# TeemoCaption/FDDM-asr

Measured on AMD Instinct MI355X. Metric: train-step utterances/sec (10 s @16 kHz, seq_len 256) at 1/2/4/8 MI355X, higher is better.
Workload: dtype bf16; 1 GPU; fddm_zhTW_base C2: WavLM-base + 6L d512 H8 ff2048 decoder, V=8000, T=200, dropout 0.1, n_step_fd=4; global_batch=32, seq_len=256, parallelism=dp1

## Files before the change

fddm-asr_amd/fddm_hip/graphs.py:

```python
from __future__ import annotations

import weakref
from types import SimpleNamespace

import torch

from . import runtime as rt


class GraphedEncoder:
    def __init__(self, encoder, nslots: int = 2):
        self._enc = weakref.ref(encoder)
        self.nslots = nslots
        self.cache: dict = {}

    @staticmethod
    def supported(encoder) -> bool:
        return getattr(encoder, "pooling", "none") == "none" and hasattr(encoder, "backbone") and \
            hasattr(encoder.backbone, "stage_rest")

    @property
    def enc(self):
        return self._enc()

    def _capture(self, wave):
        bb = self.enc.backbone
        inp = wave.detach().clone()
        h0 = bb.stage_conv0(inp)
        h1 = bb.stage_conv1(h0)
        self.enc.project(bb.stage_rest(h1))
        with rt.retaining() as keep:
            gA = torch.cuda.CUDAGraph()
            with torch.cuda.graph(gA):
                h0 = bb.stage_conv0(inp)
            h1 = torch.empty(bb.conv_out_shape(h0), device=h0.device, dtype=h0.dtype)
            gC = torch.cuda.CUDAGraph()
            with torch.cuda.graph(gC, pool=gA.pool()):
                out = self.enc.project(bb.stage_rest(h1))
        return SimpleNamespace(inp=inp, h0=h0, h1=h1, out=out, gA=gA, gC=gC, keep=keep)

    def _weights_token(self):
        enc = self.enc
        P = enc.backbone._prepared(rt.compute_dtype())
        proj = getattr(enc, "proj", None)
        pw = getattr(proj, "weight", None) if getattr(enc, "use_proj", False) else None
        return (id(P), None if pw is None else (pw.data_ptr(), pw._version), rt.cache_epoch()), P

    @torch.no_grad()
    def run(self, wave, slot: int, cap: int = 0):
        tok, P = self._weights_token()
        if tok != getattr(self, "_tok", None):
            self.cache.clear()
            self._tok, self._P = tok, P
        key = (tuple(wave.shape), wave.dtype, str(wave.device), rt.precision(), int(cap),
               int(getattr(self.enc.backbone, "conv_cus", 0)),
               int(getattr(self.enc.backbone, "conv_cus_rest", 0)))
        slots = self.cache.setdefault(key, [None] * self.nslots)
        s = slots[slot]
        if s is None:
            s = slots[slot] = self._capture(wave)
        s.inp.copy_(wave, non_blocking=True)
        s.gA.replay()
        self.enc.backbone.stage_conv1(s.h0, out=s.h1)
        s.gC.replay()
        return s.out


class StepGraphs:

    def __init__(self, device):
        self.device = torch.device(device)
        self.graphs: dict = {}
        self.static: dict = {}
        self.pool = None
        self.off = torch.zeros(1, device=self.device, dtype=torch.int64)

    def reset(self):
        self.graphs.clear()
        self.static.clear()
        self.pool = None

    @staticmethod
    def _hparams(optimizer):
        return tuple((float(g.get("lr", 0.0)), float(g.get("weight_decay", 0.0)),
                      tuple(float(b) for b in g.get("betas", ())), float(g.get("eps", 0.0)))
                     for g in getattr(optimizer, "param_groups", ()))

    def _token(self, params, optimizer, step_args):
        return (rt.cache_epoch(), getattr(optimizer, "table_epoch", 0), self._hparams(optimizer), tuple(step_args),
                tuple((p.data_ptr(), p._version) for p in params))

    def get(self, kind, params, optimizer, shapes, step_args=()):
        s = self.graphs.get(kind)
        if s is None:
            return None
        if s.shapes != shapes or s.token != self._token(params, optimizer, step_args):
            self.reset()
            return None
        return s

    def capture(self, kind, fn, inputs: dict, params, optimizer, step_args=()):
        from ._lib import lib
        shapes = tuple((k, tuple(v.shape), v.dtype) for k, v in sorted(inputs.items()))
        if any(self.static.get(k) is None or self.static[k].shape != v.shape or self.static[k].dtype != v.dtype
               for k, v in inputs.items()):
            self.reset()
            self.static = {k: torch.empty_like(v) for k, v in inputs.items()}
        for k, v in inputs.items():
            self.static[k].copy_(v)
        c0 = rt.seed_counter()
        g = torch.cuda.CUDAGraph()
        with rt.retaining() as keep:
            lib().fddm_set_seed_offset(self.off.data_ptr())
            try:
                with torch.cuda.graph(g, pool=self.pool):
                    outs = fn(**self.static)
            finally:
                lib().fddm_set_seed_offset(None)
        nseeds = rt.seed_counter() - c0
        rt.set_seed_counter(c0)
        if self.pool is None:
            self.pool = g.pool()
        self.graphs[kind] = SimpleNamespace(g=g, outs=outs, c0=c0, nseeds=nseeds, keep=keep, shapes=shapes,
                                            token=self._token(params, optimizer, step_args))

    def replay(self, kind, inputs: dict):
        s = self.graphs[kind]
        for k, v in inputs.items():
            self.static[k].copy_(v, non_blocking=True)
        c = rt.seed_counter()
        self.off.fill_(c - s.c0)
        rt.set_seed_counter(c + s.nseeds)
        s.g.replay()
        return s.outs
```

fddm-asr_amd/fddm_hip/runtime.py:

```python
from __future__ import annotations

import contextlib
import math
import os

import weakref

import torch

from . import ops

_precision = os.environ.get("FDDM_PRECISION", "bf16")


def precision() -> str:
    return _precision


def set_precision(p: str) -> None:
    global _precision
    if p not in ("bf16", "fp32"):
        raise ValueError(p)
    _precision = p

# ... 145 lines not shown


def set_seed_counter(c: int) -> None:
    global _seed_counter
    _seed_counter = int(c)


def reseed(seed: int) -> None:
    global _base_seed, _seed_counter
    _base_seed = int(seed) & 0xFFFFFFFF
    _seed_counter = 0


def seed_state() -> list:
    return [-1 if _base_seed is None else int(_base_seed), int(_seed_counter)]


def set_seed_state(state) -> None:
    global _base_seed, _seed_counter
    b, c = int(state[0]), int(state[1])
    _base_seed = None if b < 0 else b
    _seed_counter = c


_tables: dict = {}


def _table_get(k, owner):
    v = _tables.get(k)
    return _retain(v[1]) if v is not None and v[0]() is owner else None


def _table_put(k, owner, t):
    _tables[k] = (weakref.ref(owner), _retain(t))


def rope_tables(L: int, inv_freq: torch.Tensor, device):
    k = ("rope", L, id(inv_freq), inv_freq._version, inv_freq.numel(), str(device))
    t = _table_get(k, inv_freq)
    if t is None:
        f = inv_freq.detach().float().cpu()
        pos = torch.arange(L, dtype=f.dtype)
        fr = torch.outer(pos, f)
        emb = torch.cat((fr, fr), dim=-1)
        t = (emb.cos().contiguous().to(device), emb.sin().contiguous().to(device))
        _table_put(k, inv_freq, t)
    return t


def rel_bucket(rel: torch.Tensor, num_buckets: int, max_distance: int) -> torch.Tensor:
    nb = num_buckets // 2
    buckets = (rel > 0).to(torch.long) * nb
    rel = torch.abs(rel)
    max_exact = nb // 2
    is_small = rel < max_exact
    large = torch.log(rel.float() / max_exact)
    large = large / math.log(max_distance / max_exact)
    large = large * (nb - max_exact)
    large = (max_exact + large).to(torch.long)
    large = torch.min(large, torch.full_like(large, nb - 1))
    return buckets + torch.where(is_small, rel, large)


def relbias_table(S: int, embed: torch.Tensor, num_buckets: int, max_distance: int):
    k = ("rel", S, id(embed), embed._version, num_buckets, max_distance)
    t = _table_get(k, embed)
    if t is None:
        rel = torch.arange(-(S - 1), S)
        b = rel_bucket(rel, num_buckets, max_distance).to(embed.device)
        t = embed.detach().float()[b].t().contiguous()
        _table_put(k, embed, t)
    return t


class GradArena:

    ALIGN = 64

    def __init__(self, params, order=None):
        self.params = [p for p in params if p.requires_grad]
        if not self.params:
            raise ValueError("empty grad arena")
        if order is not None:
            rank = {id(p): i for i, p in enumerate(order)}
            self.params.sort(key=lambda p: rank.get(id(p), len(rank)))
        offs, n = [], 0
        for p in self.params:
            offs.append(n)
            n += (p.numel() + self.ALIGN - 1) // self.ALIGN * self.ALIGN
        dev = self.params[0].device
        self.flat = torch.zeros(n, device=dev, dtype=torch.float32)
        self.offs = offs + [n]
        self.slot = {id(p): i for i, p in enumerate(self.params)}
        self.on_ready = None
        self.reducer = None
        self.clean = False
        self.views = []
        for p, o in zip(self.params, offs):
            v = self.flat[o:o + p.numel()].view_as(p)
            self.views.append(v)
            p._fddm_arena = self
        self.attach()

    def attach(self):
        for p, v in zip(self.params, self.views):
            if p.grad is None or p.grad.data_ptr() != v.data_ptr():
                p.grad = v

    def zero_(self):
        self.attach()
        self.flat.zero_()


def grads_ready(params) -> None:
    for p in params:
        a = getattr(p, "_fddm_arena", None)
        if a is not None and a.on_ready is not None:
            a.on_ready(params)
            return


def grad_slot(p: torch.Tensor):
    a = getattr(p, "_fddm_arena", None)
    g = p.grad
    if a is None or g is None or g.dtype != torch.float32:
        return None
    return g


_probes: dict | None = None
_replay_n = 0


@contextlib.contextmanager
def probe(name: str, replay=None):
    if _probes is None or name not in _probes:
        yield
        return
    s = torch.cuda.current_stream()
    e0, e1 = torch.cuda.Event(enable_timing=True), torch.cuda.Event(enable_timing=True)
    e0.record(s)
    yield
    e1.record(s)
    _probes[name].append((e0, e1))
    if replay is not None and _replay_n > 0:
        r0, r1 = torch.cuda.Event(enable_timing=True), torch.cuda.Event(enable_timing=True)
        r0.record(s)
        for _ in range(_replay_n):
            replay()
        r1.record(s)
        _probes.setdefault(name + "#replay", []).append((r0, r1, _replay_n))


def probing_any(prefix: str) -> bool:
    return _probes is not None and any(n.startswith(prefix) for n in _probes)


@contextlib.contextmanager
def probing(names, replays=0):
    global _probes, _replay_n
    old, old_n = _probes, _replay_n
    _probes = {n: [] for n in names}
    _replay_n = replays
    try:
        yield _probes
    finally:
        _probes, _replay_n = old, old_n
```

fddm-asr_amd/train.py:

```python
from __future__ import annotations

import argparse
import logging
import os
import random
import time
import weakref
from dataclasses import dataclass
from datetime import datetime

import torch
import yaml

from fddm.sched.diffusion_scheduler import DiscreteDiffusionScheduler
from fddm_hip import dist as fdist
from fddm_hip import functions as FN
from fddm_hip import runtime as rt
from fddm_hip._lib import lib as _fddm_lib
from fddm_hip.graphs import GraphedEncoder, StepGraphs
from fddm_hip.optim import FusedAdamW
from losses.fddm_losses import lfd_loss
from models.acoustic_encoder import AcousticEncoder
from models.denoise_decoder import DenoisingTransformerDecoder
from models.projection import SpeechProjector, TextEmbedding, TextProjector

try:
    from tqdm import tqdm
except Exception:
    tqdm = None


@dataclass
class Config:
    seed: int
    data: dict
    model: dict
    diffusion: dict
    inference: dict
    optim: dict
    lfd: dict
    log: dict


class SchedulerAdapter:

    def __init__(self, scheduler):
        self.sch = scheduler

    def sample_q(self, x0: torch.Tensor, t: torch.Tensor) -> torch.Tensor:
        if hasattr(self.sch, "sample_xt"):
            return self.sch.sample_xt(x0, t, rt.next_seed())
        B, L = x0.shape
        onehot = torch.zeros(B, L, self.sch.K, device=x0.device)
        onehot.scatter_(-1, x0.unsqueeze(-1), 1.0)
        p = self.sch.q_sample(onehot, t)
        return torch.multinomial(p.view(-1, self.sch.K), 1).view(B, L)

    def kl_term(self, xt, x0, logits_x0, t, x_mask=None) -> torch.Tensor:
        if not hasattr(self.sch, "betas"):
            raise ValueError("scheduler must provide betas [T] to build the posterior")
        mask = None
        if x_mask is not None:
            mask = x_mask.contiguous().view(torch.uint8) if x_mask.dtype == torch.bool else \
                (x_mask != 0).contiguous().view(torch.uint8)
            mask = mask.reshape(-1)
        betas = self.sch.betas
        if betas.device != logits_x0.device or betas.dtype != torch.float32:
            betas = betas.to(logits_x0.device).float().contiguous()
        return FN.KLFn.apply(logits_x0.float(), xt, x0, t, mask, betas)

    def w_t(self, t: torch.Tensor) -> torch.Tensor:
        if hasattr(self.sch, "alpha_bar"):
            return self.sch.alpha_bar.to(t.device)[t - 1]
        if hasattr(self.sch, "w_prefix"):
            return self.sch.w_prefix.to(t.device)[t - 1]
        if hasattr(self.sch, "betas"):
            cp = torch.cumprod(1.0 - self.sch.betas.to(t.device), 0)
            return cp[t - 1]
        return torch.ones_like(t, dtype=torch.float32)


def align_speech(z_speech: torch.Tensor, L: int) -> torch.Tensor:
    S = z_speech.size(1)
    if S >= L:
        return z_speech[:, :L, :]
    return torch.cat([z_speech, z_speech[:, -1:, :].repeat(1, L - S, 1)], dim=1)


def cu_caps(dev) -> dict:
    ncu = torch.cuda.get_device_properties(dev).multi_processor_count
    coll = int(os.environ.get("FDDM_COLL_CUS", 0))
    enc = int(os.environ.get("FDDM_ENC_CUS", ncu * 3 // 4))
    conv = int(os.environ.get("FDDM_ENC_CUS_CONV", ncu // 2))
    conv_rest = int(os.environ.get("FDDM_ENC_CUS_CONV2", conv))
    low = lambda c: max(8, c - coll)
    return {"enc": low(enc), "conv": low(conv), "conv_rest": low(conv_rest), "coll": coll, "ncu": ncu}


def _encoded(encoder, loader, device, optimizer):
    opt_ids = set(id(p) for g in optimizer.param_groups for p in g["params"])
    frozen = not any(id(p) in opt_ids for p in encoder.parameters())
    dev = torch.device(device)
    if dev.type != "cuda" or not frozen or os.environ.get("FDDM_NO_ENC_PIPELINE"):
        bb = getattr(encoder, "backbone", None)
        if bb is not None and getattr(bb, "conv_cus", 0):
            bb.conv_cus = bb.conv_cus_rest = 0
        for wave, x0, *rest in loader:
            wave = wave.to(device, non_blocking=True)
            x0 = x0.to(device, non_blocking=True)
            if rest and rest[0] is not None:
                c, c_mask, _ = encoder(wave, rest[0].to(device, non_blocking=True))
            else:
                c, c_mask, _ = encoder(wave)
            yield c, c_mask, x0
        return
    main = torch.cuda.current_stream(dev)
    side = _enc_stream(dev)
    caps = cu_caps(dev)
    enc_cus, conv_cus = caps["enc"], caps["conv"]
    bb = getattr(encoder, "backbone", None)
    if bb is not None and hasattr(bb, "stage_rest"):
        bb.conv_cus = conv_cus
        bb.conv_cus_rest = caps["conv_rest"]
    graphs = None
    if os.environ.get("FDDM_ENC_GRAPH", "1") != "0" and GraphedEncoder.supported(encoder):
        graphs = _ENC_GRAPHS.get(encoder)
        if graphs is None:
            graphs = _ENC_GRAPHS[encoder] = GraphedEncoder(encoder)
    nbatch = [0]

    def launch(batch):
        wave, x0, *rest = batch
        wave = wave.to(device, non_blocking=True)
        x0 = x0.to(device, non_blocking=True)
        lengths = rest[0].to(device, non_blocking=True) if rest and rest[0] is not None else None
        side.wait_stream(main)
        prev = _fddm_lib().fddm_gemm_persistent_cap(enc_cus)
        try:
            with torch.cuda.stream(side):
                if lengths is not None:
                    c, c_mask, _ = encoder(wave, lengths)
                elif graphs is not None:
                    c, c_mask = graphs.run(wave, nbatch[0] % 2, enc_cus), None
                else:
                    c, c_mask, _ = encoder(wave)
            nbatch[0] += 1
        finally:
            _fddm_lib().fddm_gemm_persistent_cap(prev)
        with torch.cuda.stream(side):
            ev = torch.cuda.Event()
            ev.record(side)
        wave.record_stream(side)
        if lengths is not None:
            lengths.record_stream(side)
        return c, c_mask, x0, ev

    it = iter(loader)
    nxt = next(it, None)
    pending = launch(nxt) if nxt is not None else None
    while pending is not None:
        c, c_mask, x0, ev = pending
        main.wait_event(ev)
        c.record_stream(main)
        if c_mask is not None:
            c_mask.record_stream(main)
        nxt = next(it, None)
        pending = launch(nxt) if nxt is not None else None
        yield c, c_mask, x0


LAST_ENQUEUE_DONE = 0.0
CLIP_MAX_NORM = 5.0
_STEP_GRAPHS = weakref.WeakKeyDictionary()
ALLREDUCE_TAIL: list | None = None


def _mark_allreduce_tail(start=None):
    if ALLREDUCE_TAIL is None or fdist.world() <= 1:
        return None
    ev = torch.cuda.Event(enable_timing=True)
    ev.record()
    if start is not None:
        ALLREDUCE_TAIL.append((start, ev))
    return ev
_ENC_STREAMS: dict = {}
_ENC_GRAPHS = weakref.WeakKeyDictionary()


def _step_graph_ok(device, scaler, optimizer, arena) -> bool:
    if os.environ.get("DEBUG_HIP_FORCE_GRAPH_QUEUES", None) == "0":
        return False
    return (torch.device(device).type == "cuda" and rt.compute_dtype() == torch.bfloat16 and scaler is None and
            arena is not None and hasattr(optimizer, "clip_and_step") and not fdist.dp_active() and
            os.environ.get("FDDM_STEP_GRAPH", "0") == "1")


def _enc_stream(dev):
    s = _ENC_STREAMS.get(dev)
    if s is None:
        s = _ENC_STREAMS[dev] = torch.cuda.Stream(dev)
    return s


def train_one_epoch(encoder, decoder, s_proj, t_embed, t_proj, scheduler, loader, optimizer, device, cfg,
                    global_step, scaler=None, epoch=1, print_epoch_summary=True, draw_t=None):
    encoder.eval()
    decoder.train()
    s_proj.train()
    t_embed.train()
    t_proj.train()
    pad_id = cfg.data["pad_id"]
    T_total = cfg.diffusion["T"]
    log_every = max(1, int(cfg.log.get("log_every", 50)))
    n_step_fd = cfg.lfd["n_step_fd"]
    tau = cfg.lfd.get("tau", 1.0)
    lambda_off = cfg.lfd["lambda_offdiag"]
    trainable = list(decoder.parameters()) + list(s_proj.parameters()) + list(t_embed.parameters()) + \
        list(t_proj.parameters())
    if getattr(optimizer, "arena", 1) is None:
        opt_ids = set(id(p) for g in optimizer.param_groups for p in g["params"])
        dparams = [p for p in decoder.parameters() if p.requires_grad]
        if all(id(p) in opt_ids for p in dparams):
            order = decoder.grad_ready_order() if hasattr(decoder, "grad_ready_order") else None
            optimizer.use_grad_arena(dparams, order)
    if fdist.dp_active() and not getattr(optimizer, "_fddm_replicas_synced", False):
        fdist.broadcast_params(trainable + list(encoder.parameters()) + list(encoder.buffers()) +
                               [b for m in (decoder, s_proj, t_embed, t_proj) for b in m.buffers()])
        optimizer._fddm_replicas_synced = True
    arena = getattr(optimizer, "arena", None)
    if arena is not None and fdist.dp_active() and arena.reducer is None:
        fdist.OverlapReducer(arena)
    lfd_group = fdist.default_group() if (fdist.dp_active() and cfg.lfd.get("sync_batch_stats", False)) else None
    pbar = loader
    if tqdm is not None and print_epoch_summary:
        pbar = tqdm(loader, desc=f"Epoch {epoch} [train]", leave=False)
    loss_sum = torch.zeros((), device=device)
    nsteps = 0
    aux = [p for m in (s_proj, t_embed, t_proj) for p in m.parameters() if p.requires_grad]
    if (arena is not None and getattr(optimizer, "aux_arena", 1) is None and aux and
            all(id(p) in set(id(q) for g in optimizer.param_groups for q in g["params"]) for p in aux)):
        optimizer.use_aux_arena(aux)

    def step(c, c_mask, x0, t, xt, fd):
        x_mask = x0 != pad_id
        logits = decoder(xt, t, c, x_mask=x_mask, c_mask=c_mask)
        loss_diff = scheduler.kl_term(xt, x0, logits, t, x_mask)
        loss = loss_diff
        loss_fd = None
        if fd:
            L = x0.shape[1]
            z_text = t_proj(t_embed(logits))
            z_speech = align_speech(s_proj(c), L)
            w_t = scheduler.w_t(t).mean()
            if lfd_group is not None:
                w_t = fdist.global_mean(w_t, lfd_group)
                loss_fd = lfd_loss(z_speech, z_text, lambda_offdiag=lambda_off, group=lfd_group)
            else:
                loss_fd = lfd_loss(z_speech, z_text, lambda_offdiag=lambda_off)
            loss = loss + tau * w_t * loss_fd
        optimizer.zero_grad(set_to_none=True)
        if fd and hasattr(optimizer, "attach_aux"):
            optimizer.attach_aux()
        if scaler is not None:
            scaler.scale(loss).backward()
            fdist.allreduce_grads(trainable)
            scaler.unscale_(optimizer)
            torch.nn.utils.clip_grad_norm_([p for p in trainable if p.grad is not None], max_norm=CLIP_MAX_NORM)
            scaler.step(optimizer)
            scaler.update()
        else:
            loss.backward()
            fused = hasattr(optimizer, "clip_and_step")
            t_bwd = _mark_allreduce_tail()
            fdist.allreduce_grads(trainable, average=not fused)
            _mark_allreduce_tail(t_bwd)
            if fused:
                optimizer.clip_and_step(max_norm=CLIP_MAX_NORM, zero_grads=True, grad_scale=1.0 / fdist.world(),
                                        return_norm=False)
            else:
                torch.nn.utils.clip_grad_norm_([p for p in trainable if p.grad is not None], max_norm=CLIP_MAX_NORM)
                optimizer.step()
        return loss, loss_diff, loss_fd

    graphs = None
    if _step_graph_ok(device, scaler, optimizer, arena):
        graphs = _STEP_GRAPHS.get(decoder)
        if graphs is None:
            graphs = _STEP_GRAPHS[decoder] = StepGraphs(device)
    for c, c_mask, x0 in _encoded(encoder, pbar, device, optimizer):
        B, L = x0.shape
        t = draw_t(B) if draw_t is not None else torch.randint(1, T_total + 1, (B,), device=device)
        xt = scheduler.sample_q(x0, t)
        fd = global_step % n_step_fd == 0
        if graphs is not None and c_mask is None and not rt.probing_any("decoder."):
            inputs = {"c": c, "x0": x0, "t": t, "xt": xt}
            shapes = tuple((k, tuple(v.shape), v.dtype) for k, v in sorted(inputs.items()))
            step_args = (CLIP_MAX_NORM, 1.0 / fdist.world())
            if graphs.get(fd, trainable, optimizer, shapes, step_args) is not None:
                loss, loss_diff, loss_fd = graphs.replay(fd, inputs)
            else:
                loss, loss_diff, loss_fd = step(c, None, x0, t, xt, fd)
                graphs.capture(fd, lambda c, x0, t, xt: step(c, None, x0, t, xt, fd), inputs, trainable, optimizer,
                               step_args)
        else:
            loss, loss_diff, loss_fd = step(c, c_mask, x0, t, xt, fd)
        loss_sum += loss.detach()
        nsteps += 1
        if tqdm is not None and print_epoch_summary and (global_step % log_every == 0):
            post = {"step": global_step, "loss": f"{float(loss):.3f}", "diff": f"{float(loss_diff):.3f}"}
            if loss_fd is not None:
                post["lfd"] = f"{float(loss_fd):.3f}"
            pbar.set_postfix(post)
        global_step += 1
    global LAST_ENQUEUE_DONE
    LAST_ENQUEUE_DONE = time.perf_counter()
    avg = float(loss_sum) / max(1, nsteps)
    if print_epoch_summary:
        logging.info(f"[Summary] Epoch {epoch} Avg Train Loss: {avg:.4f}")
    return global_step, avg


def setup_logging():
    os.makedirs("logs", exist_ok=True)
    ts = datetime.now().strftime("%Y%m%d_%H%M%S")
    logger = logging.getLogger()
    logger.setLevel(logging.INFO)
    logger.handlers.clear()
    fmt = logging.Formatter("%(asctime)s - %(levelname)s - %(message)s")
    for h in (logging.FileHandler(os.path.join("logs", f"train_{ts}.log"), encoding="utf-8"), logging.StreamHandler()):
        h.setFormatter(fmt)
        logger.addHandler(h)


def build_models(cfg: Config, device):
    d_model = cfg.model["d_model"]
    vocab = cfg.data["vocab_size"]
    pad_id = cfg.data["pad_id"]
    encoder = AcousticEncoder(**cfg.model["encoder"], d_model=d_model).to(device)
    decoder = DenoisingTransformerDecoder(vocab_size=vocab, d_model=d_model, nhead=cfg.model["nhead"],
# ... 150 lines not shown
```

include/fddm_hip.h:

```cpp
#ifndef FDDM_HIP_H
#define FDDM_HIP_H
#ifdef __cplusplus
extern "C" {
#endif

int fddm_abi_version(void);
const char* fddm_error_string(int code);

int fddm_gemm(int dtype, int a_dtype, int a_kc, int b_kc, int epi, int out_dtype, const void* A, long lda, long Mi,
              long sAb, const void* B, long ldb, void* C, long ldc, void* C2, const float* bias, float alpha, long M,
              long N, long K, unsigned long long seed, unsigned long long stream, float drop_p, float* colsum,
              void* hip_stream);

int fddm_linear_dx_rope(const void* dy, long ldy, const void* w, long ldw, float* dx, long lddx, const float* cs,
                        const float* sn, long M, long N, long K, long L, void* hip_stream);

int fddm_gemm_persistent_cap(int cap);

int fddm_gemm_dw_grouped(int n, const void* const* dy, const long* ldy, const void* const* x, const long* ldx,
                         float* const* dw, const long* lddw, float* const* db, const long* M, const long* N,
                         const long* K, long kchunk, void* hip_stream);

int fddm_conv1d_gemm(int dtype, int epi, const void* x, long lda, long sAb, long Tin, long Cg, long cstride,
                     long cpad, const void* W, void* out, long ldc, const float* bias, long Bn, long Tout, long N,
                     long K, int groups, void* hip_stream);

int fddm_posconv_gelu(const void* x, const void* W, const float* bias, void* out, long B, long S, long E, int G,
                      int kp, void* hip_stream);

int fddm_conv0_gn_gelu(int out_dtype, const float* x, const float* w, const float* gamma, const float* beta,
                       double* ws, void* out, long B, long nsamp, long T0, int C, int K, int S, float eps,
                       void* hip_stream);

int fddm_wavlm_gate(int dtype, const void* x, const float* W, const float* bias, const float* cst, float* gate, long B,
                    long S, int H, long E, void* hip_stream);

int fddm_attn_fwd(int dtype, const void* Q, long sq, const void* K, long sk, const void* V, long sv, void* O, long so,
                  float* lse, const unsigned char* key_keep, const float* gate, const float* table, int B, int H,
                  int Lq, int Lk, float scale, float drop_p, unsigned long long seed, unsigned long long stream,
                  unsigned long long* drop_bits, int drop_bits_ready, void* hip_stream);
int fddm_attn_drop_bits(unsigned long long* out, long site_words, int nsites, int B, int H, int Lq, int Lk,
                        float drop_p, unsigned long long seed, unsigned long long stream0,
                        unsigned long long stream_step, void* hip_stream);
long fddm_attn_drop_words(int B, int H, int Lq, int Lk);
int fddm_attn_fwd_relgate(const void* Q, long sq, const void* K, long sk, const void* V, long sv, void* O, long so,
                          const void* graw, long sgr, const float* gconst, const float* table, int B, int H, int Lq,
                          int Lk, float scale, void* hip_stream);
int fddm_attn_fwd_relgate_x(const void* Q, long sq, const void* K, long sk, const void* V, long sv, void* O, long so,
                            const void* x, long sx, const float* gw, const float* gconst, const float* table, int B,
                            int H, int Lq, int Lk, float scale, void* hip_stream);
long fddm_attn_bwd_ws_floats(int B, int H, int Lq, int Lk);
int fddm_attn_bwd(int dtype, const void* Q, long sq, const void* K, long sk, const void* V, long sv, const void* O,
                  long so, const void* dO, long sdo, const float* lse, void* dQ, long sdq, void* dK, long sdk,
                  void* dV, long sdv, float* delta_ws, const unsigned char* key_keep, int B, int H, int Lq, int Lk,
                  float scale, float drop_p, unsigned long long seed, unsigned long long stream,
                  const unsigned long long* drop_bits, void* hip_stream);

int fddm_attn_fwd_kx(int dtype, const void* Q, long sq, const void* K, long sk, const void* V, long sv, void* O,
                     long so, float* lse, const unsigned char* key_keep, const int* key_len, const float* gate,
                     const float* table, int B, int H, int Lq, int Lk, float scale, float drop_p,
                     unsigned long long seed, unsigned long long stream, unsigned long long* drop_bits,
                     int drop_bits_ready, void* hip_stream);
int fddm_attn_bwd_kx(int dtype, const void* Q, long sq, const void* K, long sk, const void* V, long sv, const void* O,
                     long so, const void* dO, long sdo, const float* lse, void* dQ, long sdq, void* dK, long sdk,
                     void* dV, long sdv, float* delta_ws, const unsigned char* key_keep, const int* key_len, int B,
                     int H, int Lq, int Lk, float scale, float drop_p, unsigned long long seed,
                     unsigned long long stream, const unsigned long long* drop_bits, void* hip_stream);
int fddm_attn_fwd_relgate_x_kx(const void* Q, long sq, const void* K, long sk, const void* V, long sv, void* O,
                               long so, const void* x, long sx, const float* gw, const float* gconst,
                               const float* table, const unsigned char* key_keep, const int* key_len, int B, int H,
                               int Lq, int Lk, float scale, void* hip_stream);

int fddm_ln_fwd(int x_dtype, int y_dtype, int out_dtype, const void* x, const void* y, const float* gamma,
                const float* beta, const float* film_scale, const float* film_shift, float* out_f32, void* out_t,
                float* save_s, float* mean, float* rstd, long N, long d, long rows_per_batch, float eps, float drop_p,
                unsigned long long seed, unsigned long long stream, const float* rope_cos, const float* rope_sin,
                void* rope_out, long rope_L, void* hip_stream);
int fddm_ln_bwd(int dy_dtype, const float* dout, const float* s, const float* mean, const float* rstd,
                const float* gamma, const float* beta, const float* film_scale, float* dres, void* dy_t,
                float* dgamma, float* dbeta, float* dfilm_scale, float* dfilm_shift, long N, long d,
                long rows_per_batch, float drop_p, unsigned long long seed, unsigned long long stream,
                float* partials, void* hip_stream);
int fddm_ln_bwd_slab_rows(void);
int fddm_ln_fold(int n, const float* const* partials, const long* nslab, const long* d, float* const* dgamma,
                 float* const* dbeta, float* const* dfilm_scale, float* const* dfilm_shift,
                 const long* slabs_per_batch, void* hip_stream);

int fddm_rope_fwd(int out_dtype, const float* x, const float* cs, const float* sn, void* out, long N, long L, long d,
                  void* hip_stream);
int fddm_rope_bwd(const float* dy, const float* cs, const float* sn, float* dx, long N, long L, long d,
                  void* hip_stream);

int fddm_embed_fwd(int out_dtype, const long* tok, const float* E, const float* tbias, float* out, void* out_t, long N,
                   long L, long d, void* hip_stream);
int fddm_embed_bwd(const long* tok, const float* dx, float* dE, float* dtb, long N, long L, long d, long pad_id,
                   void* hip_stream);

int fddm_colsum(int dtype, const void* X, float* out, long M, long N, long ldx, void* hip_stream);
int fddm_cast(int src_dtype, int dst_dtype, const void* x, void* y, long n, void* hip_stream);
int fddm_transpose_bf16_mt(const long* table, long ntensors, long nblocks, void* hip_stream);

int fddm_sample_q(const long* x0, const long* t, const unsigned* thr, long* xt, long B, long L, long K,
                  unsigned long long seed, unsigned long long stream, void* hip_stream);
int fddm_kl_fwd(const float* logits, const long* xt, const long* x0, const long* t, const float* betas, float* kl_tok,
                long N, long L, long V, void* hip_stream);
int fddm_kl_bwd(const float* logits, const long* xt, const long* x0, const long* t, const float* betas,
                const float* w, const float* gscale, void* dz, int dz_dtype, long N, long L, long V,
                void* hip_stream);
int fddm_kl_fused(const float* logits, const long* xt, const long* x0, const long* t, const float* betas,
                  const unsigned char* mask, float* kl_tok, void* dz, int dz_dtype, long N, long L, long V,
                  void* hip_stream);
int fddm_scale_if(void* x, int dtype, const float* g, long n, void* hip_stream);
int fddm_softmax_bwd_add_bf16(const void* y, const void* dy, const void* add, void* out, long N, long V,
                              void* hip_stream);
int fddm_axpy_if_bf16(void* x, const void* y, const float* g, long n, void* hip_stream);

int fddm_softmax_rows(const float* x, void* y, int out_dtype, long N, long V, void* hip_stream);
int fddm_softmax_bwd_rows(const void* y, const void* dy, float* dz, int dtype, long N, long V, int accumulate,
                          void* hip_stream);

int fddm_lfd_std_fwd(int out_dtype, const float* z, void* zt, float* inv_std, long B, long C, float eps,
                     void* hip_stream);
int fddm_lfd_std_bwd(int zt_dtype, const float* dzt, const void* zt, const float* inv_std, float* dz, long B, long C,
                     void* hip_stream);
int fddm_lfd_loss(const float* Cm, float* loss, long D, float lam, void* hip_stream);
int fddm_lfd_dloss(int out_dtype, const float* Cm, const float* gscale, void* dC, long D, float lam, void* hip_stream);
int fddm_lfd_colstat(const float* z, float* out, const float* mean_sum, float inv_n, long B, long C, void* hip_stream);
int fddm_lfd_std_apply(int out_dtype, const float* z, void* zt, float* inv_std, const float* s1, const float* s2,
                       float inv_n, float eps, long B, long C, void* hip_stream);
int fddm_lfd_bwd_colstat(int zt_dtype, const float* dzt, const void* zt, float* out, long B, long C, void* hip_stream);
int fddm_lfd_std_bwd_apply(int zt_dtype, const float* dzt, const void* zt, const float* inv_std, const float* sums,
                           float inv_n, float scale, float* dz, long B, long C, void* hip_stream);

int fddm_gemm_force_path(int path);
int fddm_gemm_last_path(void);
int fddm_attn_set_kernels(int v6);
int fddm_attn_last_path(void);


int fddm_set_seed_offset(const unsigned long long* off);

int fddm_grad_sumsq(const long* chunk_tensor, const long* chunk_start, const long* numel, const float* const* g,
                    long nchunks, float* total, void* hip_stream);
int fddm_adamw(const long* chunk_tensor, const long* chunk_start, const long* numel, float* const* p,
               const float* const* g, float* const* m, float* const* v, unsigned short* const* pbf,
               float* const* step, long ntensors, long nchunks, const float* total, float max_norm, float lr,
               float lr_wd, float b1, float b2, float eps, int* skipped, int zero_g, float grad_scale,
               void* hip_stream);

int fddm_rows_mean(int dtype, const void* x, float* out, long B, long S, long d, void* hip_stream);
int fddm_time_embed(const long* t, float* emb, long B, long d, float max_steps, void* hip_stream);
int fddm_small_linear(const float* in, long ldi, int njobs, const float* const* W, const float* const* bias,
                      float* const* out, float* const* out2, long ldw, long ldo, const float* aux, long R, long N, long K,
                      int act, int transpose_w, void* hip_stream);
int fddm_small_dw(int njobs, const float* const* dy, const long* lddy, const float* const* x, const long* ldx,
                  float* const* dW, float* const* db, const long* N, const long* K, long R, void* hip_stream);
int fddm_kl_reduce(const float* kl_tok, const unsigned char* mask, float* w, float* loss, long B, long L,
                   void* hip_stream);

int fddm_key_extent(const unsigned char* key_keep, long B, long Lk, int* key_len, void* hip_stream);
int fddm_rows_mean_masked(int dtype, const void* x, const unsigned char* key_keep, float* out, long B, long S, long d,
                          int clamp_count, void* hip_stream);
int fddm_rows_zero_masked(int dtype, void* x, const unsigned char* key_keep, long R, long E, void* hip_stream);

int fddm_jump(const float* logits, long ldz, const long* xt, const float* coef, long* x_next, long* x0hat, long N,
              long L, long V, int mode, float temperature, unsigned long long seed, unsigned long long stream,
              void* hip_stream);

#ifdef __cplusplus
}
#endif
#endif
```

Before: 3525 utterances/s.

## Run frozen WavLM encoder forward as a native C++ plan instead of HIP graphs

Adds a native entry point that runs the whole frozen WavLM encoder forward (conv0+GN, the remaining conv layers, feature projection, positional conv, transformer layers and projection) from a single C struct of pointers and a preallocated workspace. It is enabled by default in place of the HIP-graph replay path. The goal is to drop the Python and PyTorch per-op dispatch and graph bookkeeping, and possibly let buffers be reused more tightly. In exchange, many kernel launches are now issued from host C++ rather than replayed from a graph, and the path only covers unpadded bf16 batches with specific geometry.

```diff
diff --git a/fddm-asr_amd/csrc/wavlm_plan.hip b/fddm-asr_amd/csrc/wavlm_plan.hip
--- /dev/null
+++ b/fddm-asr_amd/csrc/wavlm_plan.hip
@@ -0,0 +1,191 @@
+#include "common.h"
+#pragma clang diagnostic push
+#pragma clang diagnostic ignored "-Wcomment"
+#include "../../include/fddm_hip.h"
+#pragma clang diagnostic pop
+
+namespace {
+
+constexpr int kBF16 = 1;
+constexpr int kEpiStore = 0, kEpiGeluOnly = 3;
+constexpr long kAlign = 256;
+
+inline long up(long bytes) { return (bytes + kAlign - 1) / kAlign * kAlign; }
+inline bool misaligned(const void* p) { return ((uintptr_t)p & 15) != 0; }
+
+const char* geometry_error(const FddmWavlmPlan* p) {
+  if (p->struct_bytes != (long)sizeof(FddmWavlmPlan)) return "plan: struct_bytes is not this library's sizeof(FddmWavlmPlan)";
+  if (p->B <= 0 || p->nsamp <= 0) return "plan: empty batch";
+  if (p->n_conv < 2 || p->n_conv > FDDM_WAVLM_MAX_CONV) return "plan: 2 .. FDDM_WAVLM_MAX_CONV conv layers";
+  if (p->conv_kernel[0] != 10 || p->conv_dim[0] % 512) return "plan: conv layer 0 is kernel 10 with a multiple of 512 channels";
+  long t = p->nsamp;
+  for (int i = 0; i < p->n_conv; ++i) {
+    if (p->conv_kernel[i] <= 0 || p->conv_stride[i] <= 0 || p->conv_dim[i] <= 0 || p->conv_dim[i] % 8)
+      return "plan: conv kernels and strides are positive, channel counts multiples of 8";
+    if (t < p->conv_kernel[i]) return "plan: an utterance shorter than the conv stack's receptive field";
+    t = (t - p->conv_kernel[i]) / p->conv_stride[i] + 1;
+    if (p->frames[i] != t) return "plan: frames[i] is not (frames[i-1] - kernel[i]) / stride[i] + 1";
+  }
+  if (p->H <= 0 || p->E != p->H * 64) return "plan: head_dim must be 64";
+  if (p->FF <= 0 || p->FF % 8) return "plan: FF width is a positive multiple of 8";
+  if (p->n_layers < 0) return "plan: negative layer count";
+  if (p->d_model < 0 || p->d_model % 8) return "plan: d_model is 0 (no projection) or a multiple of 8";
+  const int G = p->pos_groups, kp = p->pos_kernel;
+  if (G <= 0 || p->E % G || (p->E / G) % 16 || p->E / G > 64 || kp <= 0 || kp % 2)
+    return "plan: the positional conv needs E / groups a multiple of 16 up to 64 and an even tap count";
+  if (t > 0x7fffffffL / 2 || p->B > 0x7fffffffL / p->H) return "plan: B, H or the frame count exceeds the attention kernels' int range";
+  return nullptr;
+}
+
+struct Ws {
+  long gn, conv_a, conv_b, hn, x0, pos, xa, x1, o, y, qkv, hh, total;
+};
+
+Ws layout(const FddmWavlmPlan* p) {
+  Ws w{};
+  long off = 0;
+  auto take = [&](long bytes) { const long at = off; off += up(bytes); return at; };
+  const long K0 = p->conv_kernel[0];
+  const long nb = (p->frames[0] + 4095) / 4096;
+  w.gn = take((p->B * nb * (K0 + K0 * (K0 + 1) / 2) + p->B * p->conv_dim[0]) * 8);
+  long a = 0, b = 0;
+  for (int i = 2; i < p->n_conv; ++i) {
+    const long bytes = p->B * p->frames[i] * p->conv_dim[i] * 2;
+    if (i % 2 == 0) a = bytes > a ? bytes : a; else b = bytes > b ? bytes : b;
+  }
+  w.conv_a = take(a);
+  w.conv_b = take(b);
+  const long M = p->B * p->frames[p->n_conv - 1], E = p->E;
+  w.hn = take(M * p->conv_dim[p->n_conv - 1] * 2);
+  w.x0 = take(M * E * 2);
+  w.pos = take(M * E * 2);
+  w.xa = take(M * E * 2);
+  w.x1 = take(M * E * 2);
+  w.o = take(M * E * 2);
+  w.y = take(M * E * 2);
+  w.qkv = take(M * 3 * E * 2);
+  w.hh = take(M * (long)p->FF * 2);
+  w.total = off;
+  return w;
+}
+
+const char* plan_error(const FddmWavlmPlan* p, int stage) {
+  if (!p) return "plan: null";
+  if (stage != 0 && stage != 1) return "stage: 0 (conv layer 0) or 1 (everything after conv layer 1)";
+  if (const char* g = geometry_error(p)) return g;
+  if (p->key_keep || p->key_len) return "plan: a key-padding mask is not covered (padded batches take the Python path)";
+  if (!p->ws || misaligned(p->ws)) return "plan: ws is null or not 16-byte aligned";
+  if (stage == 0) {
+    if (!p->wave || !p->h0 || !p->conv0_w || !p->gn_g || !p->gn_b) return "plan: stage 0 needs wave, h0, conv0_w, gn_g, gn_b";
+    if (misaligned(p->wave) || misaligned(p->h0)) return "plan: wave / h0 not 16-byte aligned";
+    return nullptr;
+  }
+  if (!p->h1 || !p->out) return "plan: stage 1 needs h1 and out";
+  if (misaligned(p->h1) || misaligned(p->out)) return "plan: h1 / out not 16-byte aligned";
+  for (int i = 2; i < p->n_conv; ++i)
+    if (!p->conv_w[i] || misaligned(p->conv_w[i])) return "plan: conv_w[i] null or not 16-byte aligned";
+  if (!p->fp_ln_g || !p->fp_ln_b || !p->fp_w || !p->fp_b || !p->pos_w || !p->pos_b || !p->enc_ln_g || !p->enc_ln_b ||
+      !p->rel_table)
+    return "plan: a feature-projection / positional-conv / encoder weight pointer is null";
+  if (misaligned(p->fp_w) || misaligned(p->pos_w) || misaligned(p->pos_b)) return "plan: fp_w / pos_w / pos_b not 16-byte aligned";
+  if (p->d_model > 0 && (!p->proj_w || !p->proj_b || misaligned(p->proj_w))) return "plan: proj_w / proj_b null or not 16-byte aligned";
+  if (p->n_layers > 0 && !p->layers) return "plan: layers is null";
+  for (int l = 0; l < p->n_layers; ++l) {
+    const FddmWavlmLayer& L = p->layers[l];
+    if (!L.qkv_w || !L.qkv_b || !L.o_w || !L.o_b || !L.gate_w || !L.gate_const || !L.ln1_g || !L.ln1_b || !L.ff1_w ||
+        !L.ff1_b || !L.ff2_w || !L.ff2_b || !L.ln2_g || !L.ln2_b)
+      return "plan: a transformer layer's weight pointer is null";
+    if (misaligned(L.qkv_w) || misaligned(L.o_w) || misaligned(L.ff1_w) || misaligned(L.ff2_w) || misaligned(L.gate_w))
+      return "plan: a transformer layer's GEMM or gate weight is not 16-byte aligned";
+  }
+  return nullptr;
+}
+
+int linear(const void* x, const void* w, const float* bias, void* y, long M, long N, long K, int epi, void* s) {
+  return fddm_gemm(kBF16, kBF16, 1, 1, epi, kBF16, x, K, 0, 0, w, K, y, N, nullptr, bias, 1.f, M, N, K, 0, 0, 0.f, nullptr,
+                   s);
+}
+
+int ln(const void* x, const void* y, const float* g, const float* b, void* out, long N, long d, float eps, void* s) {
+  return fddm_ln_fwd(kBF16, kBF16, kBF16, x, y, g, b, nullptr, nullptr, nullptr, out, nullptr, nullptr, nullptr, N, d, 0,
+                     eps, 0.f, 0, 0, nullptr, nullptr, nullptr, 0, s);
+}
+
+int stage0(const FddmWavlmPlan* p, const Ws& w, void* s) {
+  char* ws = (char*)p->ws;
+  return fddm_conv0_gn_gelu(kBF16, p->wave, p->conv0_w, p->gn_g, p->gn_b, (double*)(ws + w.gn), p->h0, p->B, p->nsamp,
+                            p->frames[0], p->conv_dim[0], p->conv_kernel[0], p->conv_stride[0], p->gn_eps, s);
+}
+
+int conv_layers(const FddmWavlmPlan* p, const Ws& w, const void** h_out, void* s) {
+  char* ws = (char*)p->ws;
+  const void* h = p->h1;
+  for (int i = 2; i < p->n_conv; ++i) {
+    const long cin = p->conv_dim[i - 1], T = p->frames[i - 1], co = p->conv_dim[i], Tout = p->frames[i];
+    void* out = ws + (i % 2 == 0 ? w.conv_a : w.conv_b);
+    const int e = fddm_conv1d_gemm(kBF16, kEpiGeluOnly, h, cin, T * cin, T, cin, p->conv_stride[i], 0, p->conv_w[i], out, co,
+                                   nullptr, p->B, Tout, co, p->conv_kernel[i] * cin, 1, s);
+    if (e) return e;
+    h = out;
+  }
+  *h_out = h;
+  return 0;
+}
+
+int layers(const FddmWavlmPlan* p, const Ws& w, const void* h, void* s) {
+  char* ws = (char*)p->ws;
+  const long S = p->frames[p->n_conv - 1], M = p->B * S, E = p->E, cin = p->conv_dim[p->n_conv - 1];
+  void *hn = ws + w.hn, *x0 = ws + w.x0, *pos = ws + w.pos, *xa = ws + w.xa, *x1 = ws + w.x1, *o = ws + w.o, *y = ws + w.y,
+       *hh = ws + w.hh;
+  char* qkv = ws + w.qkv;
+  void* x = (p->n_layers == 0 && p->d_model == 0) ? p->out : xa;
+  int e;
+  if ((e = ln(h, nullptr, p->fp_ln_g, p->fp_ln_b, hn, M, cin, p->ln_eps, s))) return e;
+  if ((e = linear(hn, p->fp_w, p->fp_b, x0, M, E, cin, kEpiStore, s))) return e;
+  if ((e = fddm_posconv_gelu(x0, p->pos_w, p->pos_b, pos, p->B, S, E, p->pos_groups, p->pos_kernel, s))) return e;
+  if ((e = ln(x0, pos, p->enc_ln_g, p->enc_ln_b, x, M, E, p->ln_eps, s))) return e;
+  for (int l = 0; l < p->n_layers; ++l) {
+    const FddmWavlmLayer& L = p->layers[l];
+    if ((e = linear(x, L.qkv_w, L.qkv_b, qkv, M, 3 * E, E, kEpiStore, s))) return e;
+    if ((e = fddm_attn_fwd_relgate_x(qkv, 3 * E, qkv + E * 2, 3 * E, qkv + 2 * E * 2, 3 * E, o, E, x, E, L.gate_w,
+                                     L.gate_const, p->rel_table, (int)p->B, p->H, (int)S, (int)S, 0.125f, s)))
+      return e;
+    if ((e = linear(o, L.o_w, L.o_b, y, M, E, E, kEpiStore, s))) return e;
+    if ((e = ln(x, y, L.ln1_g, L.ln1_b, x1, M, E, p->ln_eps, s))) return e;
+    if ((e = linear(x1, L.ff1_w, L.ff1_b, hh, M, p->FF, E, kEpiGeluOnly, s))) return e;
+    if ((e = linear(hh, L.ff2_w, L.ff2_b, y, M, E, p->FF, kEpiStore, s))) return e;
+    x = (l == p->n_layers - 1 && p->d_model == 0) ? p->out : xa;
+    if ((e = ln(x1, y, L.ln2_g, L.ln2_b, x, M, E, p->ln_eps, s))) return e;
+  }
+  if (p->d_model > 0) return linear(x, p->proj_w, p->proj_b, p->out, M, p->d_model, E, kEpiStore, s);
+  return 0;
+}
+
+struct CapScope {
+  bool set;
+  int prev;
+  explicit CapScope(int cap) : set(cap > 0), prev(0) { if (set) prev = fddm_gemm_persistent_cap(cap); }
+  ~CapScope() { if (set) fddm_gemm_persistent_cap(prev); }
+};
+
+}
+
+FDDM_API const char* fddm_wavlm_plan_check(const FddmWavlmPlan* plan, int stage) { return plan_error(plan, stage); }
+
+FDDM_API long fddm_wavlm_ws_bytes(const FddmWavlmPlan* plan) {
+  if (!plan || geometry_error(plan)) return -1;
+  return layout(plan).total;
+}
+
+FDDM_API int fddm_wavlm_stage(const FddmWavlmPlan* plan, int stage, void* hip_stream) {
+  if (plan_error(plan, stage)) return (int)hipErrorInvalidValue;
+  const Ws w = layout(plan);
+  if (stage == 0) return stage0(plan, w, hip_stream);
+  const void* h = nullptr;
+  {
+    CapScope cap(plan->cap_conv);
+    if (const int e = conv_layers(plan, w, &h, hip_stream)) return e;
+  }
+  CapScope cap(plan->cap_layers);
+  return layers(plan, w, h, hip_stream);
+}
diff --git a/fddm-asr_amd/fddm_hip/graphs.py b/fddm-asr_amd/fddm_hip/graphs.py
--- a/fddm-asr_amd/fddm_hip/graphs.py
+++ b/fddm-asr_amd/fddm_hip/graphs.py
@@ -1,5 +1,7 @@
 from __future__ import annotations
 
+import ctypes
+import sys
 import weakref
 from types import SimpleNamespace
 
@@ -63,6 +65,162 @@
         s.gA.replay()
         self.enc.backbone.stage_conv1(s.h0, out=s.h1)
         s.gC.replay()
+        return s.out
+
+
+_MAX_CONV = 8
+
+
+class WavlmLayer(ctypes.Structure):
+    _fields_ = [(n, ctypes.c_void_p) for n in ("qkv_w", "qkv_b", "o_w", "o_b", "gate_w", "gate_const", "ln1_g", "ln1_b",
+                                               "ff1_w", "ff1_b", "ff2_w", "ff2_b", "ln2_g", "ln2_b")]
+
+
+class WavlmPlan(ctypes.Structure):
+    _fields_ = [("struct_bytes", ctypes.c_long), ("B", ctypes.c_long), ("nsamp", ctypes.c_long), ("n_conv", ctypes.c_int),
+                ("conv_dim", ctypes.c_int * _MAX_CONV), ("conv_kernel", ctypes.c_int * _MAX_CONV),
+                ("conv_stride", ctypes.c_int * _MAX_CONV), ("frames", ctypes.c_long * _MAX_CONV),
+                ("E", ctypes.c_int), ("H", ctypes.c_int), ("FF", ctypes.c_int), ("n_layers", ctypes.c_int),
+                ("pos_kernel", ctypes.c_int), ("pos_groups", ctypes.c_int), ("d_model", ctypes.c_int),
+                ("ln_eps", ctypes.c_float), ("gn_eps", ctypes.c_float), ("cap_conv", ctypes.c_int),
+                ("cap_layers", ctypes.c_int)] + \
+               [(n, ctypes.c_void_p) for n in ("wave", "h0", "h1", "out", "ws", "key_keep", "key_len", "conv0_w", "gn_g",
+                                               "gn_b")] + \
+               [("conv_w", ctypes.c_void_p * _MAX_CONV)] + \
+               [(n, ctypes.c_void_p) for n in ("fp_ln_g", "fp_ln_b", "fp_w", "fp_b", "pos_w", "pos_b", "enc_ln_g",
+                                               "enc_ln_b", "rel_table", "proj_w", "proj_b")] + \
+               [("layers", ctypes.POINTER(WavlmLayer))]
+
+    def ws_bytes(self) -> int:
+        from ._lib import lib
+        return int(lib().fddm_wavlm_ws_bytes(ctypes.addressof(self)))
+
+
+def wavlm_plan_geometry(config, B: int, nsamp: int, d_model: int = 0, cap_conv: int = 0, cap_layers: int = 0) -> WavlmPlan:
+    c = config
+    p = WavlmPlan()
+    p.struct_bytes = ctypes.sizeof(WavlmPlan)
+    p.B, p.nsamp, p.n_conv = B, nsamp, len(c.conv_dim)
+    if p.n_conv > _MAX_CONV:
+        raise ValueError(f"more than {_MAX_CONV} conv layers")
+    t = nsamp
+    for i, (co, k, s) in enumerate(zip(c.conv_dim, c.conv_kernel, c.conv_stride)):
+        t = (t - k) // s + 1
+        p.conv_dim[i], p.conv_kernel[i], p.conv_stride[i], p.frames[i] = co, k, s, t
+    p.E, p.H, p.FF, p.n_layers = c.hidden_size, c.num_attention_heads, c.intermediate_size, c.num_hidden_layers
+    p.pos_kernel, p.pos_groups = c.num_conv_pos_embeddings, c.num_conv_pos_embedding_groups
+    p.d_model = d_model
+    p.ln_eps, p.gn_eps = c.layer_norm_eps, 1e-5
+    p.cap_conv, p.cap_layers = cap_conv, cap_layers
+    return p
+
+
+def wavlm_plan_check(plan, stage: int):
+    from ._lib import lib
+    msg = lib().fddm_wavlm_plan_check(ctypes.addressof(plan) if plan is not None else None, stage)
+    return None if msg is None else msg.decode()
+
+
+class NativeEncoder:
+
+    MAX_SHAPES = 4
+
+    def __init__(self, encoder, nslots: int = 2):
+        self._enc = weakref.ref(encoder)
+        self.nslots = nslots
+        self.cache: dict = {}
+
+    @staticmethod
+    def supported(encoder) -> bool:
+        if not GraphedEncoder.supported(encoder) or rt.compute_dtype() != torch.bfloat16:
+            return False
+        bb = encoder.backbone
+        gate_mode = getattr(sys.modules.get(type(bb).__module__), "GATE_MODE", None)
+        proj = getattr(encoder, "proj", None)
+        d_model = proj.weight.shape[0] if getattr(encoder, "use_proj", False) else 0
+        if gate_mode != "x" or any(p.dtype != torch.float32 for p in encoder.parameters()):
+            return False
+        return wavlm_plan_geometry(bb.config, 1, 16000, d_model).ws_bytes() >= 0
+
+    @property
+    def enc(self):
+        return self._enc()
+
+    _weights_token = GraphedEncoder._weights_token
+
+    def _build(self, wave, cap):
+        enc = self.enc
+        bb = enc.backbone
+        c = bb.config
+        dev = wave.device
+        P = self._P
+        B, nsamp = wave.shape
+        d_model = enc.proj.weight.shape[0] if enc.use_proj else 0
+        p = wavlm_plan_geometry(c, B, nsamp, d_model, int(getattr(bb, "conv_cus_rest", getattr(bb, "conv_cus", 0))),
+                                int(cap))
+        nbytes = p.ws_bytes()
+        if nbytes < 0:
+            raise ValueError(f"NativeEncoder: {wavlm_plan_check(p, 0)}")
+        S = p.frames[p.n_conv - 1]
+        bf = dict(device=dev, dtype=torch.bfloat16)
+        h0 = torch.empty(B, p.frames[0], c.conv_dim[0], **bf)
+        h1 = torch.empty(B, p.frames[1], c.conv_dim[1], **bf)
+        out = torch.empty(B, S, d_model or c.hidden_size, **bf)
+        ws = torch.empty(nbytes, device=dev, dtype=torch.uint8)
+        with rt.retaining() as keep:
+            table = rt.relbias_table(S, bb.encoder.layers[0].attention.rel_attn_embed.weight, c.num_buckets,
+                                     c.max_bucket_distance)
+            proj_w = rt.wt(enc.proj.weight) if d_model else None
+        proj_b = enc.proj.bias.detach() if d_model else None
+        keep = list(keep) + [table, proj_w, proj_b]
+        ptr = lambda t: None if t is None else t.data_ptr()
+        p.h0, p.h1, p.out, p.ws = h0.data_ptr(), h1.data_ptr(), out.data_ptr(), ws.data_ptr()
+        p.conv0_w, p.gn_g, p.gn_b = P["w0"].data_ptr(), P["gn"][0].data_ptr(), P["gn"][1].data_ptr()
+        for i in range(2, p.n_conv):
+            p.conv_w[i] = P["conv"][i - 1].data_ptr()
+        p.fp_ln_g, p.fp_ln_b = P["fp_ln"][0].data_ptr(), P["fp_ln"][1].data_ptr()
+        p.fp_w, p.fp_b = P["fp"][0].data_ptr(), P["fp"][1].data_ptr()
+        p.pos_w, p.pos_b = P["pos"][0].data_ptr(), P["pos"][1].data_ptr()
+        p.enc_ln_g, p.enc_ln_b = P["enc_ln"][0].data_ptr(), P["enc_ln"][1].data_ptr()
+        p.rel_table, p.proj_w, p.proj_b = table.data_ptr(), ptr(proj_w), ptr(proj_b)
+        layers = (WavlmLayer * max(1, p.n_layers))()
+        for L, Lp in zip(layers, P["layers"]):
+            L.qkv_w, L.qkv_b = Lp["qkv"].data_ptr(), Lp["bqkv"].data_ptr()
+            L.o_w, L.o_b = Lp["o"][0].data_ptr(), Lp["o"][1].data_ptr()
+            L.gate_w, L.gate_const = Lp["gw"].data_ptr(), Lp["gru"][2].data_ptr()
+            L.ln1_g, L.ln1_b = Lp["ln1"][0].data_ptr(), Lp["ln1"][1].data_ptr()
+            L.ff1_w, L.ff1_b = Lp["f1"][0].data_ptr(), Lp["f1"][1].data_ptr()
+            L.ff2_w, L.ff2_b = Lp["f2"][0].data_ptr(), Lp["f2"][1].data_ptr()
+            L.ln2_g, L.ln2_b = Lp["ln2"][0].data_ptr(), Lp["ln2"][1].data_ptr()
+        p.layers = ctypes.cast(layers, ctypes.POINTER(WavlmLayer))
+        return SimpleNamespace(plan=p, addr=ctypes.addressof(p), layers=layers, h0=h0, h1=h1, out=out, ws=ws, keep=keep)
+
+    @torch.no_grad()
+    def run(self, wave, slot: int, cap: int = 0):
+        from . import ops
+        from ._lib import call
+        enc = self.enc
+        bb = enc.backbone
+        if rt.probing_any("wavlm.", exclude=("wavlm.conv1",)):
+            return enc.project(bb.stage_rest(bb.stage_conv1(bb.stage_conv0(wave))))
+        tok, P = self._weights_token()
+        if tok != getattr(self, "_tok", None):
+            self.cache.clear()
+            self._tok, self._P = tok, P
+        wave = wave.float().contiguous()
+        key = (tuple(wave.shape), str(wave.device), rt.precision(), int(cap),
+               int(getattr(bb, "conv_cus_rest", getattr(bb, "conv_cus", 0))))
+        slots = self.cache.pop(key, None) or [None] * self.nslots
+        self.cache[key] = slots
+        while len(self.cache) > self.MAX_SHAPES:
+            self.cache.pop(next(iter(self.cache)))
+        s = slots[slot]
+        if s is None:
+            s = slots[slot] = self._build(wave, cap)
+        s.plan.wave = wave.data_ptr()
+        call("fddm_wavlm_stage", s.addr, 0, ops.stream())
+        bb.stage_conv1(s.h0, out=s.h1)
+        call("fddm_wavlm_stage", s.addr, 1, ops.stream())
         return s.out
 
 
diff --git a/fddm-asr_amd/fddm_hip/runtime.py b/fddm-asr_amd/fddm_hip/runtime.py
--- a/fddm-asr_amd/fddm_hip/runtime.py
+++ b/fddm-asr_amd/fddm_hip/runtime.py
@@ -321,8 +321,8 @@
         _probes.setdefault(name + "#replay", []).append((r0, r1, _replay_n))
 
 
-def probing_any(prefix: str) -> bool:
-    return _probes is not None and any(n.startswith(prefix) for n in _probes)
+def probing_any(prefix: str, exclude=()) -> bool:
+    return _probes is not None and any(n.startswith(prefix) and n not in exclude for n in _probes)
 
 
 @contextlib.contextmanager
diff --git a/fddm-asr_amd/train.py b/fddm-asr_amd/train.py
--- a/fddm-asr_amd/train.py
+++ b/fddm-asr_amd/train.py
@@ -17,7 +17,7 @@
 from fddm_hip import functions as FN
 from fddm_hip import runtime as rt
 from fddm_hip._lib import lib as _fddm_lib
-from fddm_hip.graphs import GraphedEncoder, StepGraphs
+from fddm_hip.graphs import GraphedEncoder, NativeEncoder, StepGraphs
 from fddm_hip.optim import FusedAdamW
 from losses.fddm_losses import lfd_loss
 from models.acoustic_encoder import AcousticEncoder
@@ -124,9 +124,11 @@
         bb.conv_cus_rest = caps["conv_rest"]
     graphs = None
     if os.environ.get("FDDM_ENC_GRAPH", "1") != "0" and GraphedEncoder.supported(encoder):
-        graphs = _ENC_GRAPHS.get(encoder)
+        native = os.environ.get("FDDM_ENC_NATIVE", "1") != "0" and NativeEncoder.supported(encoder)
+        cache, cls = (_ENC_NATIVE, NativeEncoder) if native else (_ENC_GRAPHS, GraphedEncoder)
+        graphs = cache.get(encoder)
         if graphs is None:
-            graphs = _ENC_GRAPHS[encoder] = GraphedEncoder(encoder)
+            graphs = cache[encoder] = cls(encoder)
     nbatch = [0]
 
     def launch(batch):
@@ -185,6 +187,7 @@
     return ev
 _ENC_STREAMS: dict = {}
 _ENC_GRAPHS = weakref.WeakKeyDictionary()
+_ENC_NATIVE = weakref.WeakKeyDictionary()
 
 
 def _step_graph_ok(device, scaler, optimizer, arena) -> bool:
diff --git a/include/fddm_hip.h b/include/fddm_hip.h
--- a/include/fddm_hip.h
+++ b/include/fddm_hip.h
@@ -163,6 +163,62 @@
                           int clamp_count, void* hip_stream);
 int fddm_rows_zero_masked(int dtype, void* x, const unsigned char* key_keep, long R, long E, void* hip_stream);
 
+#define FDDM_WAVLM_MAX_CONV 8
+typedef struct {
+  const void* qkv_w;
+  const float* qkv_b;
+  const void* o_w;
+  const float* o_b;
+  const float* gate_w;
+  const float* gate_const;
+  const float* ln1_g;
+  const float* ln1_b;
+  const void* ff1_w;
+  const float* ff1_b;
+  const void* ff2_w;
+  const float* ff2_b;
+  const float* ln2_g;
+  const float* ln2_b;
+} FddmWavlmLayer;
+typedef struct {
+  long struct_bytes;
+  long B, nsamp;
+  int n_conv;
+  int conv_dim[FDDM_WAVLM_MAX_CONV], conv_kernel[FDDM_WAVLM_MAX_CONV], conv_stride[FDDM_WAVLM_MAX_CONV];
+  long frames[FDDM_WAVLM_MAX_CONV];
+  int E, H, FF, n_layers;
+  int pos_kernel, pos_groups;
+  int d_model;
+  float ln_eps, gn_eps;
+  int cap_conv, cap_layers;
+  const float* wave;
+  void* h0;
+  const void* h1;
+  void* out;
+  void* ws;
+  const unsigned char* key_keep;
+  const int* key_len;
+  const float* conv0_w;
+  const float* gn_g;
+  const float* gn_b;
+  const void* conv_w[FDDM_WAVLM_MAX_CONV];
+  const float* fp_ln_g;
+  const float* fp_ln_b;
+  const void* fp_w;
+  const float* fp_b;
+  const void* pos_w;
+  const float* pos_b;
+  const float* enc_ln_g;
+  const float* enc_ln_b;
+  const float* rel_table;
+  const void* proj_w;
+  const float* proj_b;
+  const FddmWavlmLayer* layers;
+} FddmWavlmPlan;
+const char* fddm_wavlm_plan_check(const FddmWavlmPlan* plan, int stage);
+long fddm_wavlm_ws_bytes(const FddmWavlmPlan* plan);
+int fddm_wavlm_stage(const FddmWavlmPlan* plan, int stage, void* hip_stream);
+
 int fddm_jump(const float* logits, long ldz, const long* xt, const float* coef, long* x_next, long* x0hat, long N,
               long L, long V, int mode, float temperature, unsigned long long seed, unsigned long long stream,
               void* hip_stream);
```

Measured after the change: 3527 utterances/s (median of 2 runs). Within noise of the previous version (+0.1%).
